# chenxuhao/caffe-escoin

Measured on AMD Instinct MI355X. Metric: conv-layer fwd images/sec, higher is better.
Workload: dtype f32

## Files before the change

### caffe-escoin_amd/csrc/align_rules.cpp

```cpp
#include "align_rules.h"

#include <algorithm>
#include <cmath>
#include <cstdio>
#include <cstdlib>

#include "knobs.h"

namespace escoin {

constexpr int kDefaultDenseThresholdPct = 50;
constexpr int kGenericDenseThresholdPct = 4;

std::vector<char> dense_groups(const Geometry &g, const std::vector<long> &nnz_per_group, const SplitOptions &o, int n_cu) {
  const int G = g.d.group;
  std::vector<char> dense(G, 0);
  const double per_group = (double)g.Mg * g.kdim;
  long nnz = 0;
  for (long n_g : nnz_per_group) nnz += n_g;
  if (o.kernel == ESCOIN_KERNEL_DENSE || o.conv_mode == ESCOIN_CONV_MODE_LOWERED_GEMM) {
    dense.assign(G, 1);
  } else if (o.kernel == ESCOIN_KERNEL_AUTO) {
    if (o.dense_gate) {
      if ((double)nnz_per_group[0] / per_group > 0.2) dense.assign(G, 1);
// ... 123 lines not shown
  s.epi_store = (size_t)n_images * g.d.M * t.OH * t.OW * 4 < ((size_t)1 << 31);
  s.grid_y = groups * t.n_ocblk;
  const int wg_per_cu = std::max(1, 8 / t.waves);
  const int gx = std::max(1, (n_cu * wg_per_cu) / s.grid_y);
  s.grid_x = std::min(s.tiles, gx);
  static const int xm = (int)ESC_KNOB("XCD_MAP", -1);
  static const long min_code_env = ESC_KNOB_SET("XCD_MIN_CODE_KB") ? ESC_KNOB("XCD_MIN_CODE_KB", 0) * 1024 : -1;
  const long min_code = min_code_env >= 0 ? min_code_env : 2l << 20;
  const int nwg = s.grid_x * s.grid_y;
  const bool on = s.grid_y > 1 && nwg >= 8 && (xm == 1 || (xm < 0 && jit && code_bytes >= min_code));
  s.xcd_q = on ? nwg / 8 : -1;
  s.xcd_r = on ? nwg % 8 : 0;
  return s;
}

JitLayout jit_layout(const Geometry &g, float density, int tiling_batch, int n_cu) {
  JitLayout lay;
  ConvGeom cg = to_geom(g);
  cg.density = density;
  static const int env_jit_nbuf = (int)ESC_KNOB("JIT_NBUF", 0);
  int jit_nbuf = env_jit_nbuf == 2 || env_jit_nbuf == 3 ? env_jit_nbuf
                 : (g.d.KH == 1 && g.d.KW == 1 && density <= 0.101f && g.Mg <= 384) ? 3 : 2;
  int jit_budget = jit_nbuf == 3 ? std::min(default_lds_budget(), 48 * 1024) : default_lds_budget();
  Tiling t = pick_tiling(g, n_cu, jit_budget, density, tiling_batch, true);
  if (!t.ok) return lay;
  if (!ESC_KNOB_SET("LDS_KB") && g.d.KH * g.d.KW > 1 && t.n_ocblk > 1 && jit_nbuf == 2 && jit_budget > 32 * 1024) {
    const Tiling t32 = pick_tiling(g, n_cu, 32 * 1024, density, tiling_batch, true);
    if (t32.ok) {
      t = t32;
      jit_budget = 32 * 1024;
// ... 390 lines not shown
```

### caffe-escoin_amd/csrc/align_rules.h

```cpp
#ifndef ESCOIN_ALIGN_RULES_H_
#define ESCOIN_ALIGN_RULES_H_

#include <string>
#include <vector>

#include "geometry.h"
#include "jit_codegen.h"
#include "stream_builder.h"

namespace escoin {

constexpr int kTiledWaves = 8;
constexpr int kLdsBudget = 64 * 1024;

typedef std::vector<std::vector<int>> CsrIndex;
typedef std::vector<std::vector<float>> CsrValues;

struct SplitOptions {
  int kernel, conv_mode, dense_gate, dense_threshold_pct, tiling_batch;
};
std::vector<char> dense_groups(const Geometry &g, const std::vector<long> &nnz_per_group, const SplitOptions &o, int n_cu);

struct GroupSplit {
  int n_dense = 0, n_sparse = 0;
// ... 20 lines not shown
  bool strided = false;
  int n_dense_groups = 0;
  bool epi_store = false;
  long workgroups = 0;
};
int body_variant(const Geometry &g, const Tiling &t, const BodyLaunch &l, int option);

struct TiledLaunchShape {
  int tiles = 0;
  int grid_x = 0, grid_y = 0;
  int xcd_q = -1, xcd_r = 0;
  bool epi_store = false;
};
TiledLaunchShape tiled_launch_shape(const Geometry &g, const Tiling &t, int n_images, int groups, bool jit, long code_bytes,
                                    int n_cu);

struct JitLayout {
  bool ok = false;
  Tiling t;
  int nbuf = 2;
  int budget = 0;
  int tab_len = 0;
  jit::Options jopt;
};
JitLayout jit_layout(const Geometry &g, float density, int tiling_batch, int n_cu);
bool jit_generate(const Geometry &g, float density, int tiling_batch, int n_cu, JitLayout *lay, const CsrIndex &rowptr,
                  const CsrIndex &colidx, const CsrValues &values, jit::Program *prog);

struct StreamLayout {
  bool ok = false;
// ... 134 lines not shown
```

### caffe-escoin_amd/csrc/escoin_capi.hip

```cpp
#include <hip/hip_runtime.h>

#include <algorithm>
#include <chrono>
#include <cstring>
#include <new>
#include <string>
#include <vector>

#include "align_rules.h"
#include "aligned_form.h"
#include "escoin_plan.h"
#include "prune_rules.h"

namespace escoin {

static thread_local std::string g_last_error;

S2dHooks g_s2d_hooks = {nullptr, nullptr, nullptr};
S2bHooks g_s2b_hooks = {nullptr, nullptr, nullptr, nullptr};
B2sHooks g_b2s_hooks = {nullptr, nullptr, nullptr, nullptr};

void set_error(const std::string &msg) { g_last_error = msg; }

int fail(int code, const std::string &msg) {
// ... 579 lines not shown
    if (!strcmp(key, "wgrad_channel_block")) {
      if (value < 0) return fail(ESCOIN_EINVAL, "wgrad_channel_block must be >= 0");
      p->wgrad_channel_block = value;
      return ESCOIN_OK;
    }
    if (!strcmp(key, "dense_wgrad_splits")) {
      if (value < 0) return fail(ESCOIN_EINVAL, "dense_wgrad_splits must be >= 0");
      p->dense_wgrad_splits = value;
      return ESCOIN_OK;
    }
    if (!strcmp(key, "body_variant")) {
      if (value < -1 || value > 0) return fail(ESCOIN_EINVAL, "body_variant must be -1 (automatic) or 0 (generic)");
      p->body_variant = value;
      return ESCOIN_OK;
    }
    if (!strcmp(key, "stream_stores")) {
      if (value < -1 || value > 1) return fail(ESCOIN_EINVAL, "stream_stores must be -1, 0 or 1");
      p->stream_stores = value;
      return ESCOIN_OK;
    }
    if (!strcmp(key, "kernel")) {
      if (value < ESCOIN_KERNEL_AUTO || value > ESCOIN_KERNEL_JIT)
        return fail(ESCOIN_EINVAL, "unknown kernel id");
      p->kernel_choice = value;
    } else if (!strcmp(key, "conv_mode")) {
      if (value < ESCOIN_CONV_MODE_LOWERED_GEMM || value > ESCOIN_CONV_MODE_SCONV_PAR)
        return fail(ESCOIN_EINVAL, "conv_mode must be one of Caffe::ConvMode's four values (0..3)");
      auto direct = [](int m) { return m == ESCOIN_CONV_MODE_SCONV || m == ESCOIN_CONV_MODE_SCONV_PAR; };
      const bool regroup = p->aligned && ((value == ESCOIN_CONV_MODE_LOWERED_GEMM) != (p->conv_mode == ESCOIN_CONV_MODE_LOWERED_GEMM) ||
                                          ((p->s2d || p->s2b || p->b2s) && !p->is_f64 && direct(value) != direct(p->conv_mode)));
// ... 141 lines not shown
}

long escoin_plan_stat(const escoin_plan *p, const char *key) {
  if (!p || !key) return fail(ESCOIN_EINVAL, "null argument");
  if (!strcmp(key, "s2d")) return p->s2d_state ? 1 : 0;
  if (!strcmp(key, "s2d_scratch_bytes")) return p->s2d_state ? (long)p->s2d_state->x.bytes() : 0;
  if (!strcmp(key, "s2b")) return p->s2b_state ? 1 : 0;
  if (!strcmp(key, "s2b_scratch_bytes")) return p->s2b_state ? (long)(p->s2b_state->x.bytes() + p->s2b_state->t.bytes()) : 0;
  if (!strcmp(key, "b2s")) return p->b2s_state ? 1 : 0;
  if (!strcmp(key, "b2s_block")) return p->b2s_state ? p->b2s_state->bp.B : 0;
  if (!strcmp(key, "b2s_scratch_bytes"))
    return p->b2s_state ? (long)(p->b2s_state->x.bytes() + p->b2s_state->t.bytes() + p->b2s_state->dx.bytes()) : 0;
  if (p->inner_plan()) {
    static const char *const inner_keys[] = {"kernel_choice", "code_bytes", "code_direct", "small_launch_rule", "jit_rows", "jit_records",
                                             "deal_slowest_over_mean_x1000", "deal_worst_block_x1000", "lds_bytes", "body_variant",
                                             "workgroup_columns", "streamk_gave_up", "streamk", "dense_variant"};
    for (const char *k : inner_keys)
      if (!strcmp(key, k)) return escoin_plan_stat(p->inner_plan()->plan.get(), key);
  }
  if (!strcmp(key, "align_us")) return (long)(p->align_ms * 1e3);
  if (!strcmp(key, "code_bytes")) return (long)(p->tiled.enabled && p->tiled.jit ? p->tiled_dev.jit.code_bytes : 0);
  if (!strcmp(key, "device_bytes")) return (long)device_bytes(p).fwd;
  if (!strcmp(key, "import_fast")) return p->import_fast ? 1 : 0;
  if (!strcmp(key, "cpu_images_per_job")) return p->cpu_img_last;
  if (!strcmp(key, "cpu_channel_block")) return p->cpu_blk_cb;
  if (!strcmp(key, "code_direct")) return p->tiled_dev.jit.direct ? 1 : 0;
  if (!strcmp(key, "small_launch_rule")) return p->small_rule;
  if (!strcmp(key, "jit_rows")) return p->tiled.jit ? p->tiled.jit_rows : 0;
  if (!strcmp(key, "jit_records")) return p->tiled.jit ? p->tiled.jit_records : 0;
  if (!strcmp(key, "deal_slowest_over_mean_x1000")) return p->tiled.jit ? (long)(p->tiled.deal_slowest_over_mean * 1000.f + 0.5f) : 0;
  if (!strcmp(key, "deal_worst_block_x1000")) return p->tiled.jit ? (long)(p->tiled.deal_worst_block * 1000.f + 0.5f) : 0;
  if (!strcmp(key, "lds_bytes")) return p->tiled.enabled ? (long)p->tiled.lds_bytes : 0;
  if (!strcmp(key, "body_variant")) return p->tiled.enabled ? p->tiled.body_variant_last : 0;
  if (!strcmp(key, "workgroup_columns")) return p->tiled.enabled ? p->tiled.tiling.n_ocblk : 0;
  if (!strcmp(key, "streamk_gave_up")) {
    const DenseArrays &dn = p->dense;
    if (!dn.sk_ws.get<void>() || dn.sk_flag_words < 1 || !dn.sk_used) return 0;
    if (dn.sk_fail.host() && *(volatile unsigned *)dn.sk_fail.host() != 0u) return 1;
    unsigned v = 0;
    if (hipMemcpy(&v, dn.sk_ws.get<const unsigned>() + (dn.sk_flag_words - 1), 4, hipMemcpyDeviceToHost) != hipSuccess)
      return fail(ESCOIN_EHIP, "streamk_gave_up: device read failed");
    return (long)v;
  }
  if (!strcmp(key, "streamk")) return p->dense.sk_used ? 1 : 0;
  if (!strcmp(key, "dense_variant")) return p->dense.variant_last;
  if (!strncmp(key, "bwd_", 4) || !strncmp(key, "wgrad_", 6) || !strncmp(key, "dgrad_", 6)) return bwd_stat(p, key);
  if (!strncmp(key, "upd", 3)) return upd_stat(p, key);
  if (!strncmp(key, "dwg_", 4)) return dwg_stat(p, key);
// ... 196 lines not shown
```

### caffe-escoin_amd/csrc/escoin_plan.h

```cpp
#ifndef ESCOIN_PLAN_H_
#define ESCOIN_PLAN_H_

#include <hip/hip_runtime.h>

#include <chrono>
#include <memory>
#include <new>
#include <stdexcept>
#include <string>
#include <vector>

#include "csr_tables.h"
#include "device_buffer.h"
#include "align_rules.h"
#include "escoin.h"
#include "geometry.h"
#include "jit_module.h"
#include "stream_builder.h"

namespace escoin {

void set_error(const std::string &msg);
int fail(int code, const std::string &msg);
int check_plan_device(const escoin_plan *p, const std::string &who);
// ... 28 lines not shown
  size_t lds_bytes = 0;
  int lds_budget = 0;
  float density = 0.f;
  Tiling tiling;
  int stage_bytes = 0;
  int nbuf = 2;
  bool jit = false;
  long jit_rows = 0, jit_records = 0;
  bool jit_dma = false;
  int dma_period = 0;
  int jit_pref = 0;
  bool jit_chain = false;
  float deal_slowest_over_mean = 1.f, deal_worst_block = 1.f;
  std::string info;
  mutable int body_variant_last = 0;
};

struct CpuWorkspace {
  std::vector<char> pad, scratch, partial;
  const void *src = nullptr;
  unsigned long call = 0;
};

struct DerivedPlan {
  std::unique_ptr<escoin_plan, int (*)(escoin_plan *)> plan{nullptr, escoin_plan_destroy};
  std::vector<int> src;
};


struct GatherDgrad {
// ... 157 lines not shown

  escoin::GenericArrays gen;
  escoin::TiledConfig tiled;
  escoin::TiledArrays tiled_dev;
  int code_loader = 0;
  double align_ms = 0.0;
  bool import_fast = false;
  int small_rule = 0;

  escoin::DenseArrays dense;
  bool use_dense = false;
  unsigned long long dense_mask = 0, sparse_mask = ~0ull;
  int n_dense_groups = 0, n_sparse_groups = 0;
  int dense_threshold_pct = -1;
  int body_variant = -1;
  int stream_stores = -1;

  escoin::DeviceBuffer col;

  std::string kernel_name = "(not aligned)";

  int bwd_kernel = ESCOIN_KERNEL_AUTO;
  int wgrad_kernel = ESCOIN_WGRAD_AUTO;
  int wgrad_channel_block = 0;
  std::unique_ptr<escoin::BwdState> bwd;

  std::unique_ptr<escoin::UpdState> upd;
  bool dev_authoritative = false;
  int (*sync_host_fn)(escoin_plan *) = nullptr;
  hipStream_t upd_stream = nullptr;
// ... 123 lines not shown
```

### caffe-escoin_amd/csrc/sconv_tiled.hip

```cpp
#include <hip/hip_runtime.h>

#include <chrono>

#include <algorithm>
#include <cmath>
#include <atomic>
#include <cstdlib>
#include <cstring>
#include <string>
#include <type_traits>
#include <vector>

#include "align_rules.h"
#include "aligned_form.h"
#include "escoin_plan.h"
#include "jit_codegen.h"
#include "knobs.h"
#include "stream_builder.h"
#include "stream_loop_asm.inc"

namespace escoin {

struct TiledArgs {
  const float *__restrict__ in;
  float *__restrict__ out;
  const unsigned *__restrict__ stream;
  const float *__restrict__ bias;
  int n_images, C, H, W, M, OH, OW, Cg, Mg, KH, pad_h, pad_w;
  int s4_log2, rows_per_slab, pix_waves_log2, oc_waves, G, n_ocg, n_ocblk;
  int tr, nseg, band_mode, bands, plane_rows, plane_seg_floats, plane_ch_floats, icb, n_icb;
  int qpc;
  int qpc64_log2;
  int nt_planes;
  int nt_out;
  int n_tiles;
  int grid_x, nthreads;
  int xcd_q, xcd_r;
  int buf_bytes;
  int vec_in, vec_out;
  int epi_store;
  int epi5_ok;
  int relu;
  const unsigned *__restrict__ unit_hdr;
  const unsigned *__restrict__ chan;
  int stage_bytes;
  int nbuf;
  unsigned stream_bytes;
  int fill_waves;
  float inv_nseg, inv_bands, inv_qpc;
  unsigned long long *prof;
  unsigned long long group_mask;
  int hdr_stride, hdr_word;
// ... 269 lines not shown
  r[3] = 0x00020000u;
  return r;
}

template <class A>
__device__ __forceinline__ void tile_origin(const A &a, int tile, int &img0, int &y0) {
  if (a.band_mode) {
    img0 = div_small(tile, a.inv_bands);
    y0 = (tile - img0 * a.bands) * a.tr;
  } else {
    img0 = tile * a.nseg;
    y0 = 0;
  }
}

__device__ __forceinline__ void touch_first_unit(unsigned long long code_base, unsigned boff_v, int jit_pref) {
  const unsigned long long c0 = code_base + __builtin_amdgcn_readfirstlane(boff_v);
  const unsigned lane64 = (unsigned)opaque_lane() * 64u;
  for (int k = 0; k < jit_pref; ++k)
    asm volatile("global_load_dword v62, %0, %1" :: "v"(lane64 + (unsigned)k * 4096u), "s"(c0) : "v62", "memory");
}

__device__ __forceinline__ void drop_code_caches() {
  asm volatile("s_waitcnt lgkmcnt(0)\n\ts_dcache_inv\n\ts_icache_inv\n\t"
               "s_nop 0\n\ts_nop 0\n\ts_nop 0\n\ts_nop 0\n\ts_nop 0\n\ts_nop 0\n\ts_nop 0\n\ts_nop 0\n\t"
               "s_nop 0\n\ts_nop 0\n\ts_nop 0\n\ts_nop 0\n\ts_nop 0\n\ts_nop 0\n\ts_nop 0\n\ts_nop 0" ::: "memory");
}

#define ESC_CHAIN_CALL(...)                                                                                         \
  asm volatile("v_mov_b32 v32, %[lbA]\n"                                                                           \
               "v_add_u32 v33, 0x400, v32\n"                                                                       \
               "v_mov_b32 v34, %[tabv]\n"                                                                          \
               "v_lshlrev_b32 v63, 6, %[lane]\n"                                                                   \
               "s_mov_b32 s44, %[r0]\n"                                                                            \
               "s_mov_b32 s45, %[r1]\n"                                                                            \
               "s_mov_b32 s46, %[r2]\n"                                                                            \
               "s_mov_b32 s47, %[r3]\n"                                                                            \
               "s_mov_b32 s48, %[fb]\n"                                                                            \
               "s_mov_b32 s52, %[wb]\n"                                                                            \
               "s_mov_b32 s53, %[r2n]\n"                                                                           \
               "s_mov_b32 s54, %[td]\n"                                                                            \
               "s_swappc_b64 s[30:31], %[tgt]\n"                                                                   \
               :: [lbA] "v"(lbAb), [tabv] "v"(tabv), [tgt] "s"(tgt), [r0] "s"(rsrc[0]), [r1] "s"(rsrc[1]),         \
                  [r2] "s"(r2_entry), [r3] "s"(rsrc[3]), [fb] "s"(fill_base), [wb] "s"(walk_base), [r2n] "s"(r2_next), \
                  [td] "s"(tab_delta), [lane] "v"(lane_id)                                                         \
               : ESC_STREAM_LOOP_CLOBBERS, "s30", "s31", "s46", "s47", "s48", "s49", "s50", "s51", "s52", "s53", "s54", "s55" __VA_ARGS__)
template <bool kSweights>
__device__ __forceinline__ void chain_call(unsigned lbAb, unsigned tabv, unsigned long long tgt, const u32x4 &rsrc,
                                           unsigned r2_entry, unsigned fill_base, unsigned walk_base, unsigned r2_next,
                                           unsigned tab_delta, unsigned lane_id) {
  if constexpr (kSweights) ESC_CHAIN_CALL(, ESC_JIT_SW_CLOBBERS);
  else ESC_CHAIN_CALL();
}
#undef ESC_CHAIN_CALL

template <int KW, int T, int R>
struct EpiAsmK;
#define ESC_EAK_ARGS                                                                                                \
  unsigned voff, const float *base, unsigned ostr, unsigned gcnt, unsigned flags, unsigned long long ok,            \
      unsigned long long okp, float bias_v, unsigned pm, unsigned chan_v
#define ESC_EAK_OPERANDS                                                                                            \
  [voff] "v"(voff), [base] "s"(base), [ostr] "s"(ostr), [gcount] "s"(gcnt), [flags] "s"(flags), [ok] "s"(ok),       \
      [okp] "s"(okp), [bias] "v"(bias_v), [pm] "v"(pm), [chanv] "v"(chan_v)
#define ESC_EAK(T, R)                                                                                               \
  template <>                                                                                                       \
// ... 95 lines not shown
}
__device__ __forceinline__ float bias_lanes_from(float bias_v, int lane, int first) {
  return __builtin_bit_cast(float, __builtin_amdgcn_ds_bpermute(((lane + first) & 63) << 2, __builtin_bit_cast(int, bias_v)));
}

template <int KW, int PADW, bool kInWalk, bool kJit>
__device__ __forceinline__ void tiled_body(TiledArgs a) {
  extern __shared__ __attribute__((aligned(16))) float lds[];
  ESC_PROF_DECL
  const int nthreads = a.nthreads;
  const int nwaves = nthreads >> 6;
  const int wave = __builtin_amdgcn_readfirstlane((int)threadIdx.x >> 6);
  const int pw = wave & ((1 << a.pix_waves_log2) - 1);
  const int ow = wave >> a.pix_waves_log2;
  int bx = (int)blockIdx.x, by = (int)blockIdx.y;
  if (a.xcd_q >= 0) {
    const int orig = by * a.grid_x + bx;
    const int xcd = orig & 7, k = orig >> 3;
    const int wg = (xcd < a.xcd_r ? xcd * (a.xcd_q + 1) : a.xcd_r * (a.xcd_q + 1) + (xcd - a.xcd_r) * a.xcd_q) + k;
    by = wg / a.grid_x;
    bx = wg - by * a.grid_x;
  }
  const int gsel = by / a.n_ocblk;
  const int ocblk = by - gsel * a.n_ocblk;
  const int cg = a.group_mask == ~0ull ? gsel : nth_set_bit(a.group_mask, gsel);
  const int S4m = (1 << a.s4_log2) - 1;
  const int ocg = ocblk * a.oc_waves + ow;
  const bool wave_active = ocg < a.n_ocg;
  const int hw = a.in_plane;

  auto lane_quads = [&](unsigned &lbA, unsigned &lbB) {
    const int lane = opaque_lane();
    lbA = (unsigned)((pw * 64 * a.tpl + lane) * 16);
    lbB = lbA + 1024u;
  };

  const int nbuf = a.nbuf;
// ... 119 lines not shown
    chan_v = a.chan[(size_t)(cg * a.n_ocg + ocg) * a.G + (threadIdx.x & 63)];
    if (a.bias) asm volatile("s_waitcnt vmcnt(0)" : "+v"(chan_v));
  }
  float bias_v = 0.f;
  if (a.bias && wave_active && (int)(threadIdx.x & 63) < gcount) bias_v = a.bias[cg * a.Mg + chan_v];
  unsigned boff_v = 0;
  if ((int)(threadIdx.x & 63) < a.n_icb) boff_v = hdr0[(size_t)(threadIdx.x & 63) * a.hdr_stride];
  ESC_SPROF(0);
  build_tab(bx, tab0);
  ESC_SPROF(1);
  asm volatile("s_waitcnt vmcnt(0)" : "+v"(bias_v), "+v"(boff_v), "+v"(chan_v));
  ESC_SPROF(2);

  if ((int)(threadIdx.x & 63) < a.n_icb) boff_tab[threadIdx.x & 63] = boff_v;
  for (int i = 64 + (int)(threadIdx.x & 63); i < a.n_icb; i += 64) boff_tab[i] = hdr0[(size_t)i * a.hdr_stride];
  if (kJit && a.jit_pref > 0 && wave_active) touch_first_unit(a.code_base, boff_v, a.jit_pref);
  if (kJit && a.jit_prio > 0 && wave >= (nwaves >> 1) && nwaves > 1) __builtin_amdgcn_s_setprio(1);
  u32x8 h = {0, 0, 0, 0, 0, 0, 0, 0};
  ESC_SPROF(3);
  __syncthreads();
  ESC_SPROF(4);
  int f_tile = bx, f_blk = 0, f_tix = 0, f_buf = 0;
  int younger = 0;
  auto issue_next = [&]() {
    if (f_tile >= a.n_tiles) {
      younger = 0;
      return;
    }
    const unsigned bo = __builtin_amdgcn_readfirstlane(boff_tab[f_blk]);
    younger = issue_fill(tab0 + (f_tix & 1) * a.tab_len, f_blk, f_buf, bo);
    f_buf = f_buf + 1 == nbuf ? 0 : f_buf + 1;
// ... 58 lines not shown
      const unsigned cur_tab = tabs + (unsigned)((t_idx & 1) * a.tab_len * 4), nxt_tab = tabs + (unsigned)(((t_idx + 1) & 1) * a.tab_len * 4);
      const unsigned r2_next = __builtin_amdgcn_readfirstlane(has_next ? rsrc[2] : 0u);
      const unsigned r2_entry = stage_next_at_entry ? r2_next : rsrc[2];
      const unsigned tab_delta = __builtin_amdgcn_readfirstlane(nxt_tab - cur_tab);
      int fb = c_buf + ahead;
      if (fb >= nbuf) fb -= nbuf;
      const unsigned walk_base = __builtin_amdgcn_readfirstlane((unsigned)(c_buf * a.buf_bytes));
      const unsigned fill_base = __builtin_amdgcn_readfirstlane((unsigned)(fb * a.buf_bytes));
      unsigned lbAb, lbBb;
      lane_quads(lbAb, lbBb);
      lbAb += walk_base;
      const unsigned long long tgt = a.code_base + code_off;
      const unsigned lane_id = (unsigned)opaque_lane();
      const unsigned tabv = (stage_next_at_entry ? nxt_tab : cur_tab) + 4u * lane_id;
      ESC_PROF(4);
      chain_call<KW != 1>(lbAb, tabv, tgt, rsrc, r2_entry, fill_base, walk_base, r2_next, tab_delta, lane_id);
      c_buf += chain_adv;
      if (c_buf >= nbuf) c_buf -= nbuf;
      ESC_PROF(5);
    } else
    for (int blk = 0; blk < a.n_icb; ++blk) {
      ESC_PROF(1);
      if (nbuf == 2 || drain) asm volatile("s_waitcnt vmcnt(0)" ::: "memory");
      else wait_vmcnt_at_most(younger);
      drain = false;
      ESC_PROF(2);
      __syncthreads();
      const unsigned sbase = (unsigned)(stage_base + (c_buf * nwaves + wave) * a.stage_bytes);
      const unsigned code_off = kJit ? __builtin_amdgcn_readfirstlane(boff_tab[blk]) : 0u;
      if (!kJit) {
        const uint4 *hp = reinterpret_cast<const uint4 *>(reinterpret_cast<const char *>(lds) + sbase);
// ... 25 lines not shown
      ESC_PROF(4);
      if (kJit) {
        if (wave_active) {
          const unsigned pb = (unsigned)(c_buf * a.buf_bytes);
          unsigned lbAb, lbBb;
          lane_quads(lbAb, lbBb);
          lbAb += pb;
          const unsigned long long tgt = a.code_base + code_off;
          const unsigned lane_id = (unsigned)opaque_lane();
          const unsigned tabv = x_tab + 4u * lane_id;
          const unsigned r2 = __builtin_amdgcn_readfirstlane(x_have ? rsrc[2] : 0u);
#define ESC_UNIT_CALL(...)                                                                                        \
          asm volatile("v_mov_b32 v32, %[lbA]\n"                                                                   \
                       "v_add_u32 v33, 0x400, v32\n"                                                               \
                       "v_mov_b32 v34, %[tabv]\n"                                                                  \
                       "v_lshlrev_b32 v63, 6, %[lane]\n"                                                           \
                       "s_mov_b32 s44, %[r0]\n"                                                                    \
                       "s_mov_b32 s45, %[r1]\n"                                                                    \
                       "s_mov_b32 s46, %[r2]\n"                                                                    \
                       "s_mov_b32 s47, %[r3]\n"                                                                    \
                       "s_mov_b32 s48, %[fb]\n"                                                                    \
                       "s_swappc_b64 s[30:31], %[tgt]\n"                                                           \
                       :: [lbA] "v"(lbAb), [tabv] "v"(tabv), [tgt] "s"(tgt), [r0] "s"(rsrc[0]), [r1] "s"(rsrc[1]), \
                          [r2] "s"(r2), [r3] "s"(rsrc[3]), [fb] "s"(x_base), [lane] "v"(lane_id)                   \
                       : ESC_STREAM_LOOP_CLOBBERS, "s30", "s31", "s46", "s47", "s48", "s49", "s50", "s51" __VA_ARGS__)
          if (KW != 1) ESC_UNIT_CALL(, ESC_JIT_SW_CLOBBERS);
          else ESC_UNIT_CALL();
#undef ESC_UNIT_CALL
        }
      } else
      if (wave_active) {
        const unsigned pb = (unsigned)(c_buf * a.buf_bytes);
        unsigned lbAb, lbBb;
        lane_quads(lbAb, lbBb);
        lbAb += pb;
        lbBb += pb;
        const unsigned qbase = sbase + 32u;
#define ESC2_RUN_LOOP(ASM)                                                                       \
        asm volatile(ASM ::[h0] "s"(h[0]), [h1] "s"(h[1]), [h2] "s"(h[2]), [h3] "s"(h[3]),        \
// ... 158 lines not shown
  float *__restrict__ out;
  const float *__restrict__ bias;
  const unsigned *__restrict__ unit_off;
  const unsigned *__restrict__ chan;
  unsigned long long code_base;
  unsigned in_bytes;
  unsigned hw4;
  unsigned ostr;
  unsigned tabs_off;
  unsigned tab_bytes;
  int n_images, C, H, W, M, OH, OW, Cg, Mg, pad_h;
  int s4_log2, rows_per_slab, oc_waves, G, n_ocg, n_ocblk;
  int tr, nseg, band_mode, bands, icb, n_icb, qpc, tab_len, dma_chpp;
  int n_tiles, grid_x, nthreads;
  int xcd_q, xcd_r;
  int buf_bytes, nbuf, chain_adv;
  int stage_next_at_entry;
  int b_dead;
  int tpl, jit_pref, jit_prio, nt_planes, nt_out;
  unsigned flags;
  float inv_nseg, inv_bands, inv_qpc, inv_period, inv_grid_x, inv_n_ocblk;
#ifdef ESCOIN_STAMPS
  unsigned long long *prof;
#endif
};

template <int KW, int PADW>
__device__ __forceinline__ void chained_body(const ChainedArgs &a) {
  static_assert((KW == 1 && PADW == 0) || (KW == 3 && PADW == 1) || (KW == 5 && PADW == 2), "asm epilogues only");
  extern __shared__ __attribute__((aligned(16))) float lds[];
  ESC_PROF_DECL
  const int nthreads = a.nthreads;
  const int nwaves = nthreads >> 6;
  const int wave = __builtin_amdgcn_readfirstlane((int)threadIdx.x >> 6);
  int bx = (int)blockIdx.x, by = (int)blockIdx.y;
  if (a.xcd_q >= 0) {
    const int orig = by * a.grid_x + bx;
    const int xcd = orig & 7, k = orig >> 3;
    const int wg = xcd * a.xcd_q + min(xcd, a.xcd_r) + k;
    by = __builtin_amdgcn_readfirstlane(div_small(wg, a.inv_grid_x));
    bx = wg - by * a.grid_x;
  }
  const int cg = __builtin_amdgcn_readfirstlane(div_small(by, a.inv_n_ocblk));
  const int ocblk = by - cg * a.n_ocblk;
  const int S4m = (1 << a.s4_log2) - 1;
  const int ocg = ocblk * a.oc_waves + wave;

  const int nbuf = a.nbuf;
  unsigned *tab0 = reinterpret_cast<unsigned *>(reinterpret_cast<char *>(lds) + a.tabs_off);
  unsigned *boff_tab = tab0 + 2 * a.tab_len + wave * a.n_icb;
  auto build_tab = [&](int tile, unsigned *tab) {
    int img0, y0;
    tile_origin(a, tile, img0, y0);
    for (int fe = wave * 64 + opaque_lane(); fe < a.tab_len; fe += nthreads) {
      const int tch = a.tab_len > a.qpc ? div_small(fe, a.inv_qpc) : 0;
      const int fq = fe - tch * a.qpc;
      const int f_j = fq & S4m;
// ... 30 lines not shown
  const int gcount = min(a.G, a.Mg - m0);
  unsigned chan_v = (unsigned)(m0 + (int)(threadIdx.x & 63));
  if (KW != 1 && (int)(threadIdx.x & 63) < gcount) {
    chan_v = a.chan[(size_t)(cg * a.n_ocg + ocg) * a.G + (threadIdx.x & 63)];
    if (a.bias) asm volatile("s_waitcnt vmcnt(0)" : "+v"(chan_v));
  }
  float bias_v = 0.f;
  if (a.bias && (int)(threadIdx.x & 63) < gcount) bias_v = a.bias[cg * a.Mg + chan_v];
  unsigned boff_v = 0;
  if ((int)(threadIdx.x & 63) < a.n_icb) boff_v = hdr0[threadIdx.x & 63];
  ESC_SPROF(0);
  build_tab(bx, tab0);
  ESC_SPROF(1);
  asm volatile("s_waitcnt vmcnt(0)" : "+v"(bias_v), "+v"(boff_v), "+v"(chan_v));
  ESC_SPROF(2);
  if ((int)(threadIdx.x & 63) < a.n_icb) boff_tab[threadIdx.x & 63] = boff_v;
  for (int i = 64 + (int)(threadIdx.x & 63); i < a.n_icb; i += 64) boff_tab[i] = hdr0[i];
  if (a.jit_pref > 0) touch_first_unit(a.code_base, boff_v, a.jit_pref);
  if (a.jit_prio > 0 && wave >= (nwaves >> 1) && nwaves > 1) __builtin_amdgcn_s_setprio(1);
  ESC_SPROF(3);
  __syncthreads();
  ESC_SPROF(4);
  {
    int f_tile = bx, f_blk = 0, f_tix = 0, f_buf = 0;
    for (int i = 0; i + 1 < nbuf && f_tile < a.n_tiles; ++i) {
      issue_fill_x(tab0 + (f_tix & 1) * a.tab_len, f_blk, f_buf);
      f_buf = f_buf + 1 == nbuf ? 0 : f_buf + 1;
      if (++f_blk == a.n_icb) {
        f_blk = 0;
        f_tile += a.grid_x;
        ++f_tix;
      }
    }
// ... 1 lines not shown
  ESC_SPROF(5);
  if (wave == 0) drop_code_caches();
  int c_buf = 0;
  int t_idx = 0;
  for (int tile = bx; tile < a.n_tiles; tile += a.grid_x, ++t_idx) {
    const int next_tile = tile + a.grid_x;
    const bool has_next = next_tile < a.n_tiles;
    ESC_PROF(7);
    if (has_next) build_tab(next_tile, tab0 + ((t_idx + 1) & 1) * a.tab_len);
    ESC_PROF(0);
    ESC_PROF(1);
    asm volatile("s_waitcnt vmcnt(0)" ::: "memory");
    ESC_PROF(2);
    if (t_idx == 0) ESC_SPROF(6);
    __syncthreads();
    const unsigned code_off = __builtin_amdgcn_readfirstlane(boff_tab[0]);
    ESC_PROF(3);
    const unsigned cur_tab = a.tabs_off + (unsigned)(t_idx & 1) * a.tab_bytes;
    const unsigned nxt_tab = a.tabs_off + (unsigned)((t_idx + 1) & 1) * a.tab_bytes;
    const unsigned r2_next = __builtin_amdgcn_readfirstlane(has_next ? rsrc[2] : 0u);
    const unsigned r2_entry = a.stage_next_at_entry ? r2_next : rsrc[2];
    const unsigned tab_delta = __builtin_amdgcn_readfirstlane(nxt_tab - cur_tab);
    int fb = c_buf + nbuf - 1;
    if (fb >= nbuf) fb -= nbuf;
    const unsigned walk_base = __builtin_amdgcn_readfirstlane((unsigned)(c_buf * a.buf_bytes));
    const unsigned fill_base = __builtin_amdgcn_readfirstlane((unsigned)(fb * a.buf_bytes));
    const unsigned lane_id = (unsigned)opaque_lane();
    const unsigned lbAb = lane_id * 16u + walk_base;
    const unsigned long long tgt = a.code_base + code_off;
    const unsigned tabv = (a.stage_next_at_entry ? nxt_tab : cur_tab) + 4u * lane_id;
    ESC_PROF(4);
    chain_call<KW != 1>(lbAb, tabv, tgt, rsrc, r2_entry, fill_base, walk_base, r2_next, tab_delta, lane_id);
    c_buf += a.chain_adv;
    if (c_buf >= nbuf) c_buf -= nbuf;
    ESC_PROF(5);

    const int lane = opaque_lane();
    const int j = lane & S4m;
    int img0, y0;
    tile_origin(a, tile, img0, y0);
    constexpr int kGMax = ESC_NACC_TILE / (4 * KW);
    (void)kGMax;
    auto tile_ctx = [&](int tl, bool &store_ok) {
      const int fr = tl * a.rows_per_slab + (lane >> a.s4_log2);
      const int yl = div_small(fr, a.inv_nseg), seg = fr - yl * a.nseg;
      const bool in_tile = yl < a.tr;
      int n, y;
// ... 292 lines not shown

static ChainedArgs chained_args(const TiledArgs &a, dim3 grid) {
  ChainedArgs c;
  memset(&c, 0, sizeof(c));
  c.in = a.in; c.out = a.out; c.bias = a.bias; c.unit_off = a.unit_hdr; c.chan = a.chan; c.code_base = a.code_base;
  c.in_bytes = (unsigned)((size_t)a.n_images * a.C * a.in_plane * 4);
  c.hw4 = (unsigned)a.in_plane * 4u;
  c.ostr = (unsigned)((size_t)a.OH * a.out_w * 4);
  c.tabs_off = (unsigned)(a.nbuf * a.buf_bytes);
  c.tab_bytes = (unsigned)a.tab_len * 4u;
  c.n_images = a.n_images; c.C = a.C; c.H = a.H; c.W = a.W; c.M = a.M; c.OH = a.OH; c.OW = a.OW; c.Cg = a.Cg; c.Mg = a.Mg;
  c.pad_h = a.pad_h; c.s4_log2 = a.s4_log2; c.rows_per_slab = a.rows_per_slab; c.oc_waves = a.oc_waves; c.G = a.G;
  c.n_ocg = a.n_ocg; c.n_ocblk = a.n_ocblk; c.tr = a.tr; c.nseg = a.nseg; c.band_mode = a.band_mode; c.bands = a.bands;
  c.icb = a.icb; c.n_icb = a.n_icb; c.qpc = a.qpc; c.tab_len = a.tab_len; c.dma_chpp = a.dma_chpp;
  c.n_tiles = a.n_tiles; c.grid_x = a.grid_x; c.nthreads = a.nthreads; c.xcd_q = a.xcd_q; c.xcd_r = a.xcd_r;
  c.buf_bytes = a.buf_bytes; c.nbuf = a.nbuf; c.chain_adv = a.n_icb % a.nbuf;
  c.stage_next_at_entry = a.n_icb <= a.nbuf - 1 ? 1 : 0;
  c.b_dead = (a.tpl == 1 || a.tr * a.nseg <= a.rows_per_slab) ? 1 : 0;
  c.tpl = a.tpl; c.jit_pref = a.jit_pref; c.jit_prio = a.jit_prio; c.nt_planes = a.nt_planes; c.nt_out = a.nt_out;
  c.flags = (a.bias ? 1u : 0u) | (a.relu ? 2u : 0u);
  c.inv_nseg = a.inv_nseg; c.inv_bands = a.inv_bands; c.inv_qpc = a.inv_qpc; c.inv_period = a.inv_period;
  c.inv_grid_x = 1.0f / (float)grid.x; c.inv_n_ocblk = 1.0f / (float)a.n_ocblk;
#ifdef ESCOIN_STAMPS
  c.prof = a.prof;
#endif
  return c;
}

#ifdef ESCOIN_STAMPS
struct StampProfileDump {
// ... 171 lines not shown
  a.xcd_r = ls.xcd_r;
  if (grid.y > 65535u) return fail(ESCOIN_EINVAL, "tiled kernel: grid.y exceeds 65535");
  const size_t lds = lds_bytes_for(t, a.stage_bytes, a.nbuf, a.jit_dma ? a.tab_len : 0);
  if (lds > kLdsPerWorkgroup) return fail(ESCOIN_ESTATE, "tiled kernel: LDS budget exceeded");
  if ((size_t)n_images * g.d.C * g.d.H * g.d.W * 4 >= 0xFFFFFFF0ull)
    return fail(ESCOIN_ESTATE, "tiled kernel: sub-batch exceeds the descriptor range");
  const bool st = static_pad(g);
#ifdef ESCOIN_STAMPS
  StampProfileDump prof_dump{a.prof, grid.x * grid.y, stream};
#endif
  BodyLaunch bl;
  bl.jit = jit; bl.chained = a.jit_chain != 0; bl.dma_in_code = a.jit_dma != 0; bl.stage_bytes = a.stage_bytes;
  bl.strided = strided; bl.n_dense_groups = p->n_dense_groups; bl.epi_store = a.epi_store != 0;
  bl.workgroups = (long)grid.x * grid.y;
  p->tiled.body_variant_last = body_variant(g, t, bl, p->body_variant);
  const int threads = 64 * t.waves;
  if (p->tiled.body_variant_last == 1) {
    const ChainedArgs c = chained_args(a, grid);
    switch (g.d.KW) {
      case 1: return launch_kernel<escoin_sconv_jit_kernel<1, 0, true>>(c, grid, threads, lds, stream);
      case 3: return launch_kernel<escoin_sconv_jit_kernel<3, 1, true>>(c, grid, threads, lds, stream);
      default: return launch_kernel<escoin_sconv_jit_kernel<5, 2, true>>(c, grid, threads, lds, stream);
    }
  }
#define ESC_LAUNCH(K, KW, PADW) launch_kernel<K<KW, PADW>>(a, grid, threads, lds, stream)
  if (jit) switch (g.d.KW) {
    case 1: return st ? ESC_LAUNCH(escoin_sconv_jit_kernel, 1, 0) : ESC_LAUNCH(escoin_sconv_jit_kernel, 1, -1);
    case 2: return ESC_LAUNCH(escoin_sconv_jit_kernel, 2, -1);
    case 3: return st ? ESC_LAUNCH(escoin_sconv_jit_kernel, 3, 1) : ESC_LAUNCH(escoin_sconv_jit_kernel, 3, -1);
    case 4: return ESC_LAUNCH(escoin_sconv_jit_kernel, 4, -1);
// ... 19 lines not shown
```

Before: 144,000.

## Elect one workgroup per stride to prefetch JIT code lines per XCD

Adds a toucher election so only every T-th workgroup (per XCD rank) issues the per-lane code-prefetch loads that warm the instruction cache for JIT-generated code; other workgroups touch a single line. The stride is passed into the kernel, encoded into the boff table low bit for the chained variant, and fed into the JIT code's v63 lane offset. This is meant to cut redundant global loads of the code stream across many workgroups on the same XCD. The risk is that non-elected workgroups run before their XCD's shared cache is warm, and the extra scalar setup adds a little per-launch work.

```diff
diff --git a/caffe-escoin_amd/csrc/align_rules.cpp b/caffe-escoin_amd/csrc/align_rules.cpp
--- a/caffe-escoin_amd/csrc/align_rules.cpp
+++ b/caffe-escoin_amd/csrc/align_rules.cpp
@@ -161,6 +161,37 @@
   return s;
 }
 
+TouchWorkgroup touch_workgroup(const TiledLaunchShape &s, int orig, int T) {
+  TouchWorkgroup w;
+  w.xcd = orig & (kTouchXcds - 1);
+  const int k = orig >> 3;
+  const int wg = s.xcd_q >= 0 ? w.xcd * s.xcd_q + std::min(w.xcd, s.xcd_r) + k : orig;
+  w.by = wg / s.grid_x;
+  w.bx = wg - w.by * s.grid_x;
+  w.toucher = touch_elected((unsigned)touch_rank(s.xcd_q, k, w.bx), (unsigned)T, touch_mul(T));
+  return w;
+}
+
+int touch_election(const TiledLaunchShape &s, bool jit, int n_pref, int n_cu, int option) {
+  if (!jit || n_pref <= 0 || s.grid_x >= (1 << 16) || s.grid_x < 1 || s.grid_y < 1) return 1;
+  if (option >= 1) return std::min(option, kTouchMaxStride);
+  if (n_cu < 64 || n_cu % kTouchXcds != 0) return 1;
+  return kTouchRuleStride;
+}
+
+long touch_lines(const TiledLaunchShape &s, const Tiling &t, int n_pref, int T, long *touchers) {
+  long lines = 0, nt = 0;
+  if (n_pref > 0 && s.grid_x > 0)
+    for (int orig = 0; orig < s.grid_x * s.grid_y; ++orig) {
+      const TouchWorkgroup w = touch_workgroup(s, orig, T);
+      const long walked = w.bx < s.tiles ? (s.tiles - w.bx + s.grid_x - 1) / s.grid_x : 0;
+      lines += (long)t.waves * n_pref * (1 + walked * t.n_icb) * (w.toucher ? 64 : 1);
+      nt += w.toucher;
+    }
+  if (touchers) *touchers = nt;
+  return lines;
+}
+
 JitLayout jit_layout(const Geometry &g, float density, int tiling_batch, int n_cu) {
   JitLayout lay;
   ConvGeom cg = to_geom(g);
diff --git a/caffe-escoin_amd/csrc/align_rules.h b/caffe-escoin_amd/csrc/align_rules.h
--- a/caffe-escoin_amd/csrc/align_rules.h
+++ b/caffe-escoin_amd/csrc/align_rules.h
@@ -58,6 +58,20 @@
 };
 TiledLaunchShape tiled_launch_shape(const Geometry &g, const Tiling &t, int n_images, int groups, bool jit, long code_bytes,
                                     int n_cu);
+
+constexpr int kTouchXcds = 8;
+constexpr int kTouchRuleStride = 8;
+constexpr int kTouchMaxStride = 65535;
+constexpr unsigned touch_mul(int T) { return T >= 2 ? (unsigned)((1ull << 32) / (unsigned)T + 1) : 0u; }
+constexpr int touch_rank(int xcd_q, int k, int bx) { return xcd_q >= 0 ? (k < bx ? k : bx) : bx >> 3; }
+constexpr bool touch_elected(unsigned rank, unsigned T, unsigned mul) {
+  return T <= 1u || rank == (unsigned)(((unsigned long long)rank * mul) >> 32) * T;
+}
+struct TouchWorkgroup { int bx, by, xcd; bool toucher; };
+TouchWorkgroup touch_workgroup(const TiledLaunchShape &s, int orig, int T);
+
+int touch_election(const TiledLaunchShape &s, bool jit, int n_pref, int n_cu, int option);
+long touch_lines(const TiledLaunchShape &s, const Tiling &t, int n_pref, int T, long *touchers = nullptr);
 
 struct JitLayout {
   bool ok = false;
diff --git a/caffe-escoin_amd/csrc/escoin_capi.hip b/caffe-escoin_amd/csrc/escoin_capi.hip
--- a/caffe-escoin_amd/csrc/escoin_capi.hip
+++ b/caffe-escoin_amd/csrc/escoin_capi.hip
@@ -617,6 +617,11 @@
       p->body_variant = value;
       return ESCOIN_OK;
     }
+    if (!strcmp(key, "code_touchers")) {
+      if (value < 0) return fail(ESCOIN_EINVAL, "code_touchers must be 0 (the rule) or a stride >= 1");
+      p->code_touchers = value;
+      return ESCOIN_OK;
+    }
     if (!strcmp(key, "stream_stores")) {
       if (value < -1 || value > 1) return fail(ESCOIN_EINVAL, "stream_stores must be -1, 0 or 1");
       p->stream_stores = value;
@@ -788,6 +793,7 @@
   if (p->inner_plan()) {
     static const char *const inner_keys[] = {"kernel_choice", "code_bytes", "code_direct", "small_launch_rule", "jit_rows", "jit_records",
                                              "deal_slowest_over_mean_x1000", "deal_worst_block_x1000", "lds_bytes", "body_variant",
+                                             "code_touchers", "touch_lines_per_launch",
                                              "workgroup_columns", "streamk_gave_up", "streamk", "dense_variant"};
     for (const char *k : inner_keys)
       if (!strcmp(key, k)) return escoin_plan_stat(p->inner_plan()->plan.get(), key);
@@ -806,6 +812,9 @@
   if (!strcmp(key, "deal_worst_block_x1000")) return p->tiled.jit ? (long)(p->tiled.deal_worst_block * 1000.f + 0.5f) : 0;
   if (!strcmp(key, "lds_bytes")) return p->tiled.enabled ? (long)p->tiled.lds_bytes : 0;
   if (!strcmp(key, "body_variant")) return p->tiled.enabled ? p->tiled.body_variant_last : 0;
+  if (!strcmp(key, "code_touchers")) return p->tiled.enabled ? p->tiled.touch_stride_last : 1;
+  if (!strcmp(key, "touch_lines_per_launch"))
+    return p->tiled.enabled && p->tiled.jit ? touch_lines(p->tiled.launch_shape_last, p->tiled.tiling, p->tiled.jit_pref, p->tiled.touch_stride_last) : 0;
   if (!strcmp(key, "workgroup_columns")) return p->tiled.enabled ? p->tiled.tiling.n_ocblk : 0;
   if (!strcmp(key, "streamk_gave_up")) {
     const DenseArrays &dn = p->dense;
diff --git a/caffe-escoin_amd/csrc/escoin_plan.h b/caffe-escoin_amd/csrc/escoin_plan.h
--- a/caffe-escoin_amd/csrc/escoin_plan.h
+++ b/caffe-escoin_amd/csrc/escoin_plan.h
@@ -66,6 +66,8 @@
   float deal_slowest_over_mean = 1.f, deal_worst_block = 1.f;
   std::string info;
   mutable int body_variant_last = 0;
+  mutable int touch_stride_last = 1;
+  mutable TiledLaunchShape launch_shape_last;
 };
 
 struct CpuWorkspace {
@@ -253,6 +255,7 @@
   int n_dense_groups = 0, n_sparse_groups = 0;
   int dense_threshold_pct = -1;
   int body_variant = -1;
+  int code_touchers = 0;
   int stream_stores = -1;
 
   escoin::DeviceBuffer col;
diff --git a/caffe-escoin_amd/csrc/sconv_tiled.hip b/caffe-escoin_amd/csrc/sconv_tiled.hip
--- a/caffe-escoin_amd/csrc/sconv_tiled.hip
+++ b/caffe-escoin_amd/csrc/sconv_tiled.hip
@@ -36,6 +36,7 @@
   int n_tiles;
   int grid_x, nthreads;
   int xcd_q, xcd_r;
+  unsigned touch_stride, touch_mul;
   int buf_bytes;
   int vec_in, vec_out;
   int epi_store;
@@ -335,11 +336,30 @@
   }
 }
 
-__device__ __forceinline__ void touch_first_unit(unsigned long long code_base, unsigned boff_v, int jit_pref) {
+__device__ __forceinline__ void touch_first_unit(unsigned long long code_base, unsigned boff_v, int jit_pref, unsigned touch_step) {
   const unsigned long long c0 = code_base + __builtin_amdgcn_readfirstlane(boff_v);
-  const unsigned lane64 = (unsigned)opaque_lane() * 64u;
+  const unsigned lane64 = (unsigned)opaque_lane() * touch_step;
   for (int k = 0; k < jit_pref; ++k)
     asm volatile("global_load_dword v62, %0, %1" :: "v"(lane64 + (unsigned)k * 4096u), "s"(c0) : "v62", "memory");
+}
+
+__device__ __forceinline__ unsigned touch_lane_step(int xcd_q, int k, int bx, unsigned stride, unsigned mul) {
+  unsigned step, t;
+  asm volatile("s_min_i32 %[t], %[k], %[bx]\n"
+               "s_lshr_b32 %[step], %[bx], 3\n"
+               "s_cmp_ge_i32 %[xq], 0\n"
+               "s_cselect_b32 %[t], %[t], %[step]\n"
+               "s_mul_hi_u32 %[step], %[t], %[mul]\n"
+               "s_mul_i32 %[step], %[step], %[T]\n"
+               "s_sub_u32 %[t], %[t], %[step]\n"
+               "s_cmp_le_u32 %[T], 1\n"
+               "s_cselect_b32 %[t], 0, %[t]\n"
+               "s_cmp_eq_u32 %[t], 0\n"
+               "s_cselect_b32 %[step], 64, 0\n"
+               : [step] "=&s"(step), [t] "=&s"(t)
+               : [k] "s"(k), [bx] "s"(bx), [xq] "s"(xcd_q), [mul] "s"(mul), [T] "s"(stride)
+               : "scc");
+  return step;
 }
 
 __device__ __forceinline__ void drop_code_caches() {
@@ -352,7 +372,7 @@
   asm volatile("v_mov_b32 v32, %[lbA]\n"                                                                           \
                "v_add_u32 v33, 0x400, v32\n"                                                                       \
                "v_mov_b32 v34, %[tabv]\n"                                                                          \
-               "v_lshlrev_b32 v63, 6, %[lane]\n"                                                                   \
+               "v_mov_b32 v63, %[ltouch]\n"                                                                        \
                "s_mov_b32 s44, %[r0]\n"                                                                            \
                "s_mov_b32 s45, %[r1]\n"                                                                            \
                "s_mov_b32 s46, %[r2]\n"                                                                            \
@@ -364,12 +384,12 @@
                "s_swappc_b64 s[30:31], %[tgt]\n"                                                                   \
                :: [lbA] "v"(lbAb), [tabv] "v"(tabv), [tgt] "s"(tgt), [r0] "s"(rsrc[0]), [r1] "s"(rsrc[1]),         \
                   [r2] "s"(r2_entry), [r3] "s"(rsrc[3]), [fb] "s"(fill_base), [wb] "s"(walk_base), [r2n] "s"(r2_next), \
-                  [td] "s"(tab_delta), [lane] "v"(lane_id)                                                         \
+                  [td] "s"(tab_delta), [ltouch] "v"(lane_touch)                                                    \
                : ESC_STREAM_LOOP_CLOBBERS, "s30", "s31", "s46", "s47", "s48", "s49", "s50", "s51", "s52", "s53", "s54", "s55" __VA_ARGS__)
 template <bool kSweights>
 __device__ __forceinline__ void chain_call(unsigned lbAb, unsigned tabv, unsigned long long tgt, const u32x4 &rsrc,
                                            unsigned r2_entry, unsigned fill_base, unsigned walk_base, unsigned r2_next,
-                                           unsigned tab_delta, unsigned lane_id) {
+                                           unsigned tab_delta, unsigned lane_touch) {
   if constexpr (kSweights) ESC_CHAIN_CALL(, ESC_JIT_SW_CLOBBERS);
   else ESC_CHAIN_CALL();
 }
@@ -495,13 +515,17 @@
   const int pw = wave & ((1 << a.pix_waves_log2) - 1);
   const int ow = wave >> a.pix_waves_log2;
   int bx = (int)blockIdx.x, by = (int)blockIdx.y;
+  int id8 = 0;
   if (a.xcd_q >= 0) {
     const int orig = by * a.grid_x + bx;
     const int xcd = orig & 7, k = orig >> 3;
     const int wg = (xcd < a.xcd_r ? xcd * (a.xcd_q + 1) : a.xcd_r * (a.xcd_q + 1) + (xcd - a.xcd_r) * a.xcd_q) + k;
     by = wg / a.grid_x;
     bx = wg - by * a.grid_x;
-  }
+    id8 = k;
+  }
+  const unsigned touch_step = kJit ? touch_lane_step(a.xcd_q, id8, bx, a.touch_stride, a.touch_mul) : 0u;
+  (void)touch_step;
   const int gsel = by / a.n_ocblk;
   const int ocblk = by - gsel * a.n_ocblk;
   const int cg = a.group_mask == ~0ull ? gsel : nth_set_bit(a.group_mask, gsel);
@@ -651,7 +675,7 @@
 
   if ((int)(threadIdx.x & 63) < a.n_icb) boff_tab[threadIdx.x & 63] = boff_v;
   for (int i = 64 + (int)(threadIdx.x & 63); i < a.n_icb; i += 64) boff_tab[i] = hdr0[(size_t)i * a.hdr_stride];
-  if (kJit && a.jit_pref > 0 && wave_active) touch_first_unit(a.code_base, boff_v, a.jit_pref);
+  if (kJit && a.jit_pref > 0 && wave_active) touch_first_unit(a.code_base, boff_v, a.jit_pref, touch_step);
   if (kJit && a.jit_prio > 0 && wave >= (nwaves >> 1) && nwaves > 1) __builtin_amdgcn_s_setprio(1);
   u32x8 h = {0, 0, 0, 0, 0, 0, 0, 0};
   ESC_SPROF(3);
@@ -740,7 +764,7 @@
       const unsigned lane_id = (unsigned)opaque_lane();
       const unsigned tabv = (stage_next_at_entry ? nxt_tab : cur_tab) + 4u * lane_id;
       ESC_PROF(4);
-      chain_call<KW != 1>(lbAb, tabv, tgt, rsrc, r2_entry, fill_base, walk_base, r2_next, tab_delta, lane_id);
+      chain_call<KW != 1>(lbAb, tabv, tgt, rsrc, r2_entry, fill_base, walk_base, r2_next, tab_delta, lane_id * touch_step);
       c_buf += chain_adv;
       if (c_buf >= nbuf) c_buf -= nbuf;
       ESC_PROF(5);
@@ -796,7 +820,7 @@
           asm volatile("v_mov_b32 v32, %[lbA]\n"                                                                   \
                        "v_add_u32 v33, 0x400, v32\n"                                                               \
                        "v_mov_b32 v34, %[tabv]\n"                                                                  \
-                       "v_lshlrev_b32 v63, 6, %[lane]\n"                                                           \
+                       "v_mov_b32 v63, %[ltouch]\n"                                                                \
                        "s_mov_b32 s44, %[r0]\n"                                                                    \
                        "s_mov_b32 s45, %[r1]\n"                                                                    \
                        "s_mov_b32 s46, %[r2]\n"                                                                    \
@@ -804,7 +828,7 @@
                        "s_mov_b32 s48, %[fb]\n"                                                                    \
                        "s_swappc_b64 s[30:31], %[tgt]\n"                                                           \
                        :: [lbA] "v"(lbAb), [tabv] "v"(tabv), [tgt] "s"(tgt), [r0] "s"(rsrc[0]), [r1] "s"(rsrc[1]), \
-                          [r2] "s"(r2), [r3] "s"(rsrc[3]), [fb] "s"(x_base), [lane] "v"(lane_id)                   \
+                          [r2] "s"(r2), [r3] "s"(rsrc[3]), [fb] "s"(x_base), [ltouch] "v"(lane_id * touch_step)    \
                        : ESC_STREAM_LOOP_CLOBBERS, "s30", "s31", "s46", "s47", "s48", "s49", "s50", "s51" __VA_ARGS__)
           if (KW != 1) ESC_UNIT_CALL(, ESC_JIT_SW_CLOBBERS);
           else ESC_UNIT_CALL();
@@ -993,6 +1017,7 @@
   int tr, nseg, band_mode, bands, icb, n_icb, qpc, tab_len, dma_chpp;
   int n_tiles, grid_x, nthreads;
   int xcd_q, xcd_r;
+  unsigned touch_stride, touch_mul;
   int buf_bytes, nbuf, chain_adv;
   int stage_next_at_entry;
   int b_dead;
@@ -1013,13 +1038,17 @@
   const int nwaves = nthreads >> 6;
   const int wave = __builtin_amdgcn_readfirstlane((int)threadIdx.x >> 6);
   int bx = (int)blockIdx.x, by = (int)blockIdx.y;
+  int id8 = 0;
   if (a.xcd_q >= 0) {
     const int orig = by * a.grid_x + bx;
     const int xcd = orig & 7, k = orig >> 3;
     const int wg = xcd * a.xcd_q + min(xcd, a.xcd_r) + k;
     by = __builtin_amdgcn_readfirstlane(div_small(wg, a.inv_grid_x));
     bx = wg - by * a.grid_x;
-  }
+    id8 = k;
+  }
+  const unsigned touch_step = KW == 1 ? 64u : touch_lane_step(a.xcd_q, id8, bx, a.touch_stride, a.touch_mul);
+  (void)id8;
   const int cg = __builtin_amdgcn_readfirstlane(div_small(by, a.inv_n_ocblk));
   const int ocblk = by - cg * a.n_ocblk;
   const int S4m = (1 << a.s4_log2) - 1;
@@ -1080,9 +1109,9 @@
   ESC_SPROF(1);
   asm volatile("s_waitcnt vmcnt(0)" : "+v"(bias_v), "+v"(boff_v), "+v"(chan_v));
   ESC_SPROF(2);
-  if ((int)(threadIdx.x & 63) < a.n_icb) boff_tab[threadIdx.x & 63] = boff_v;
+  if ((int)(threadIdx.x & 63) < a.n_icb) boff_tab[threadIdx.x & 63] = boff_v | ((threadIdx.x & 63) == 0 ? touch_step >> 6 : 0u);
   for (int i = 64 + (int)(threadIdx.x & 63); i < a.n_icb; i += 64) boff_tab[i] = hdr0[i];
-  if (a.jit_pref > 0) touch_first_unit(a.code_base, boff_v, a.jit_pref);
+  if (a.jit_pref > 0) touch_first_unit(a.code_base, boff_v, a.jit_pref, touch_step);
   if (a.jit_prio > 0 && wave >= (nwaves >> 1) && nwaves > 1) __builtin_amdgcn_s_setprio(1);
   ESC_SPROF(3);
   __syncthreads();
@@ -1114,7 +1143,8 @@
     ESC_PROF(2);
     if (t_idx == 0) ESC_SPROF(6);
     __syncthreads();
-    const unsigned code_off = __builtin_amdgcn_readfirstlane(boff_tab[0]);
+    const unsigned code_tag = __builtin_amdgcn_readfirstlane(boff_tab[0]);
+    const unsigned code_off = code_tag & ~1u, tile_touch_step = (code_tag & 1u) << 6;
     ESC_PROF(3);
     const unsigned cur_tab = a.tabs_off + (unsigned)(t_idx & 1) * a.tab_bytes;
     const unsigned nxt_tab = a.tabs_off + (unsigned)((t_idx + 1) & 1) * a.tab_bytes;
@@ -1130,7 +1160,7 @@
     const unsigned long long tgt = a.code_base + code_off;
     const unsigned tabv = (a.stage_next_at_entry ? nxt_tab : cur_tab) + 4u * lane_id;
     ESC_PROF(4);
-    chain_call<KW != 1>(lbAb, tabv, tgt, rsrc, r2_entry, fill_base, walk_base, r2_next, tab_delta, lane_id);
+    chain_call<KW != 1>(lbAb, tabv, tgt, rsrc, r2_entry, fill_base, walk_base, r2_next, tab_delta, lane_id * tile_touch_step);
     c_buf += a.chain_adv;
     if (c_buf >= nbuf) c_buf -= nbuf;
     ESC_PROF(5);
@@ -1453,6 +1483,7 @@
   c.n_ocg = a.n_ocg; c.n_ocblk = a.n_ocblk; c.tr = a.tr; c.nseg = a.nseg; c.band_mode = a.band_mode; c.bands = a.bands;
   c.icb = a.icb; c.n_icb = a.n_icb; c.qpc = a.qpc; c.tab_len = a.tab_len; c.dma_chpp = a.dma_chpp;
   c.n_tiles = a.n_tiles; c.grid_x = a.grid_x; c.nthreads = a.nthreads; c.xcd_q = a.xcd_q; c.xcd_r = a.xcd_r;
+  c.touch_stride = a.touch_stride; c.touch_mul = a.touch_mul;
   c.buf_bytes = a.buf_bytes; c.nbuf = a.nbuf; c.chain_adv = a.n_icb % a.nbuf;
   c.stage_next_at_entry = a.n_icb <= a.nbuf - 1 ? 1 : 0;
   c.b_dead = (a.tpl == 1 || a.tr * a.nseg <= a.rows_per_slab) ? 1 : 0;
@@ -1654,6 +1685,11 @@
   bl.strided = strided; bl.n_dense_groups = p->n_dense_groups; bl.epi_store = a.epi_store != 0;
   bl.workgroups = (long)grid.x * grid.y;
   p->tiled.body_variant_last = body_variant(g, t, bl, p->body_variant);
+  p->tiled.touch_stride_last = p->tiled.body_variant_last == 1 && g.d.KW == 1 ? 1 :
+      touch_election(ls, jit, a.jit_pref, device_cus(), p->code_touchers);
+  p->tiled.launch_shape_last = ls;
+  a.touch_stride = (unsigned)p->tiled.touch_stride_last;
+  a.touch_mul = touch_mul(p->tiled.touch_stride_last);
   const int threads = 64 * t.waves;
   if (p->tiled.body_variant_last == 1) {
     const ChainedArgs c = chained_args(a, grid);
```

Result: faster. 148,400, median of 6 (+3.1%).
